# zihuixue/DynMM

Measured on AMD Instinct MI355X. Metric: images/sec fwd+bwd, 480x640 RGB-D, batch 32/GPU, higher is better.
Workload: dtype f32; 1 GPU; configs[2]: zero-grad + fwd + weighted 4-scale CE + FLOP loss + bwd + fused SGD-Nesterov update, --dynamic --global-gate soft DiffSoftmax gates tau=1; per_gpu_batch=32, global_batch=32, height=480, width=640, parallelism=dp1, launch=eager, streams=4, optimizer_in_step=fused SGD-Nesterov

## Files before the change

### dynmm_amd/csrc/common.h

```cpp
#pragma once
#include <hip/hip_runtime.h>
#include <stdint.h>
#include <stddef.h>

#include "dynmm_hip.h"

#if defined(__HIP_DEVICE_COMPILE__) && !defined(__gfx950__)
#error "libdynmm_hip is gfx950 (MI355X) code: build with --offload-arch=gfx950"
#endif

#define DYNMM_LAUNCH_CHECK()                                   \
    do {                                                       \
        hipError_t e__ = hipGetLastError();                    \
        if (e__ != hipSuccess) return -(1000 + (int)e__);      \
    } while (0)

#define DYNMM_HIP_TRY(expr)                                    \
    do {                                                       \
        hipError_t e__ = (expr);                               \
        if (e__ != hipSuccess) return -(1000 + (int)e__);      \
    } while (0)

namespace dynmm {

// ... 18 lines not shown
    return v;
}

template <typename T>
__device__ __forceinline__ T block_reduce_sum_256(T v, T* smem) {
    v = wave_reduce_sum(v);
    const int lane = threadIdx.x & 63, wave = threadIdx.x >> 6;
    __syncthreads();
    if (lane == 0) smem[wave] = v;
    __syncthreads();
    T r = T(0);
    if (threadIdx.x == 0) r = smem[0] + smem[1] + smem[2] + smem[3];
    return r;
}

__device__ __forceinline__ float sigmoid_f(float v) { return 1.f / (1.f + expf(-v)); }
__device__ __forceinline__ float swish_fwd(float v) { return v / (1.f + expf(-v)); }
__device__ __forceinline__ float hswish_fwd(float v) { return v * fminf(fmaxf(v + 3.f, 0.f), 6.f) / 6.f; }

__device__ __forceinline__ float act_fwd(float v, int act) {
    if (act == DYNMM_ACT_RELU) return v > 0.f ? v : 0.f;
    if (act == DYNMM_ACT_TANH) return tanhf(v);
    if (act == DYNMM_ACT_SWISH) return swish_fwd(v);
    if (act == DYNMM_ACT_HSWISH) return hswish_fwd(v);
    return v;
}

__device__ __forceinline__ float act_grad_pre(float z, int act) {
    if (act == DYNMM_ACT_RELU) return z > 0.f ? 1.f : 0.f;
    if (act == DYNMM_ACT_TANH) { const float t = tanhf(z); return 1.f - t * t; }
// ... 22 lines not shown
```

### dynmm_amd/csrc/norm.hip

```cpp
#include "common.h"
#include "vec.h"

namespace dynmm {

__device__ __forceinline__ size_t mask_word(int plane, int groups, int i) { return ((size_t)plane * groups + (i >> 8)) * 4; }

static inline int reduce_splits(int N, int C) {
    int s = 2048 / (C > 0 ? C : 1);
    if (s < 1) s = 1;
    if (s > N) s = N;
    return s;
}

template <int V>
__global__ void __launch_bounds__(256) bn_stats_kernel(const float* __restrict__ x,
                                                       double* __restrict__ sums,
                                                       int N, int C, int HW) {
    __shared__ float red[4];
    const int c = blockIdx.x, S = gridDim.y;
    float s1 = 0.f, s2 = 0.f;
    for (int n = blockIdx.y; n < N; n += S) {
        const float* p = x + ((size_t)n * C + c) * HW;
        float a1 = 0.f, a2 = 0.f;
        for (int i = threadIdx.x * V; i < HW; i += 256 * V) {
// ... 679 lines not shown
```

### dynmm_amd/csrc/pointwise.hip

```cpp
#include "common.h"
#include <initializer_list>
#include "vec.h"

namespace dynmm {

__device__ __forceinline__ float keep_if(float v, bool keep) { return __int_as_float(__float_as_int(v) & -(int)keep); }


static inline int plane_chunks(int HW, int chunk) { return (HW + chunk - 1) / chunk; }
constexpr int kChunk = 8192;

__global__ void __launch_bounds__(256) maxpool_fwd_kernel(const float* __restrict__ x,
                                                          float* __restrict__ y,
                                                          signed char* __restrict__ idx, int H,
                                                          int W, int Ho, int Wo) {
    const size_t plane = blockIdx.x;
    const float* xp = x + plane * H * W;
    const int HoWo = Ho * Wo;
    const int beg = blockIdx.y * kChunk, end = min(HoWo, beg + kChunk);
    for (int i = beg + threadIdx.x; i < end; i += 256) {
        const int oh = i / Wo, ow = i - oh * Wo;
        float best = -INFINITY;
        int bi = -1;
#pragma unroll
// ... 772 lines not shown
        for (int j = 0; j < V; ++j) acc[j] += v[j];
        if (n > 2) {
            vload<V>(S.p[2] + i, v);
#pragma unroll
            for (int j = 0; j < V; ++j) acc[j] += v[j];
        }
        if (n > 3) {
            vload<V>(S.p[3] + i, v);
#pragma unroll
            for (int j = 0; j < V; ++j) acc[j] += v[j];
        }
        vstore<V>(out + i, acc);
    }
}

}

using namespace dynmm;

#define ST ((hipStream_t)stream)

extern "C" int dynmm_add_n(const float* const* srcs, int n, float* out, size_t numel, void* stream) {
    (void)hipGetLastError();
    if (!srcs || !out || n < 2 || n > 4 || numel == 0) return DYNMM_EINVAL;
    AddSrcs S{};
    bool v4 = (numel % 4 == 0) && aligned16(out);
    for (int i = 0; i < n; ++i) {
        if (!srcs[i]) return DYNMM_EINVAL;
        S.p[i] = srcs[i];
        v4 = v4 && aligned16(srcs[i]);
    }
    size_t blocks = (numel / (v4 ? 4 : 1) + 255) / 256;
    if (blocks > 8192) blocks = 8192;
    if (blocks < 1) blocks = 1;
    if (v4)
        hipLaunchKernelGGL(add_n_kernel<4>, dim3((unsigned)blocks), dim3(256), 0, ST, S, n, out, numel);
    else
        hipLaunchKernelGGL(add_n_kernel<1>, dim3((unsigned)blocks), dim3(256), 0, ST, S, n, out, numel);
    DYNMM_LAUNCH_CHECK();
    return DYNMM_OK;
}

extern "C" int dynmm_batch_gather(const float* src, const int* idx, float* dst, int n_out, size_t row,
                                  void* stream) {
    (void)hipGetLastError();
    if (!src || !dst || n_out <= 0 || row == 0) return DYNMM_EINVAL;
    unsigned bx = (unsigned)((row / 4 + 255) / 256);
    if (bx > 64) bx = 64;
    if (bx < 1) bx = 1;
    if (row % 4 == 0 && aligned16(src) && aligned16(dst))
        hipLaunchKernelGGL(batch_gather_kernel<4>, dim3(bx, n_out), dim3(256), 0, ST, src, idx, dst, row);
    else
        hipLaunchKernelGGL(batch_gather_kernel<1>, dim3(bx, n_out), dim3(256), 0, ST, src, idx, dst, row);
// ... 213 lines not shown
        hipLaunchKernelGGL(axpby_bwd_reduce_kernel<1>, dim3(NC), dim3(256), 0, ST, g, xr, xd, da, db, HW);
    DYNMM_LAUNCH_CHECK();
    return DYNMM_OK;
}

extern "C" int dynmm_axpby_bwd_apply(const float* g, const float* a, const float* b, const float* ca,
                                     const float* cb, float cscale, float* dxr, float* dxd, int NC,
                                     int HW, void* stream) {
    (void)hipGetLastError();
    if (!g || !a || !b || !dxr || !dxd || NC <= 0 || HW <= 0) return DYNMM_EINVAL;
    dim3 grid(NC, plane_chunks(HW, kChunk));
    if (can_vec4(HW, {g, dxr, dxd}))
        hipLaunchKernelGGL(axpby_bwd_apply_kernel<4>, grid, dim3(256), 0, ST, g, a, b, ca, cb, cscale, dxr, dxd, HW);
    else
        hipLaunchKernelGGL(axpby_bwd_apply_kernel<1>, grid, dim3(256), 0, ST, g, a, b, ca, cb, cscale, dxr, dxd, HW);
    DYNMM_LAUNCH_CHECK();
    return DYNMM_OK;
}

namespace dynmm {

struct StemBnArgs {
    const float* go; const signed char* io;
    const float* gd; const signed char* id;
    const float* coef; const float* off; float cscale;
    const float* x; const float* mean; const float* invstd; const float* gamma; const float* beta;
    int N, C, H, W, Ho, Wo;
};

__device__ __forceinline__ void stem_gy_block(const StemBnArgs& a, size_t plane, int ar, int t, float fc, float fo,
// ... 199 lines not shown
```

### dynmm_amd/lib.py

```python
import ctypes as C
import os
import subprocess

_HERE = os.path.dirname(os.path.abspath(__file__))
LIB_PATH = os.path.join(_HERE, 'libdynmm_hip.so')
CSRC = os.path.join(_HERE, 'csrc')

ACT_NONE, ACT_RELU, ACT_TANH, ACT_SWISH, ACT_HSWISH = 0, 1, 2, 3, 4
SMOOTH_ACTS = (ACT_SWISH, ACT_HSWISH)
DYNMM_OK, DYNMM_EINVAL, DYNMM_EUNSUPPORTED, DYNMM_EWORKSPACE = 0, -1, -2, -3
ACT = {None: 0, 'none': 0, 'relu': 1, 'tanh': 2, 'swish': 3, 'silu': 3, 'hswish': 4}
LOSS_BCE_LOGITS, LOSS_L1 = 0, 1

c_f = C.c_void_p
c_i = C.c_int
c_fl = C.c_float
c_sz = C.c_size_t
c_ll = C.c_longlong


class ConvGeom(C.Structure):
    _fields_ = [(n, C.c_int) for n in ('N', 'Ci', 'H', 'W', 'Co', 'Ho', 'Wo',
                                       'KH', 'KW', 'SH', 'SW', 'PH', 'PW', 'c_split')]

# ... 80 lines not shown
    'dynmm_upsample2x_fwd': (c_i, [c_f] * 3 + [c_i] * 5 + [c_f]),
    'dynmm_upsample2x_bwd': (c_i, [c_f] * 2 + [c_i] * 5 + [c_f]),
    'dynmm_upsample2x_dw3x3_rep_fwd': (c_i, [c_f] * 5 + [c_i] * 4 + [c_f]),
    'dynmm_upsample2x_dw3x3_rep_bwd': (c_i, [c_f] * 7 + [c_i] * 4 + [c_f]),
    'dynmm_bilinear_into_fwd': (c_i, [c_f, c_f] + [c_i] * 8 + [c_f]),
    'dynmm_bilinear_into_bwd': (c_i, [c_f, c_f] + [c_i] * 8 + [c_f]),
    'dynmm_gap2_fwd': (c_i, [c_f] * 4 + [c_i, c_i, c_f]),
    'dynmm_se_coeff_fwd': (c_i, [c_f, c_f, _PP, c_f, c_i] + [c_f] * 6 + [c_i, c_i, c_i, c_f]),
    'dynmm_se_coeff_fwd_act': (c_i, [c_f, c_f, _PP, c_f, c_i] + [c_f] * 6 + [c_i, c_i, c_i, c_i, c_f]),
    'dynmm_se_coeff_bwd_act': (c_i, [c_f] * 4 + [_PP, c_f, c_i] + [c_f] * 4 + [_PP, c_f, c_f, c_f, c_i, c_f, c_i, c_i, c_i, c_i, c_f]),
    'dynmm_se_coeff_bwd_workspace_bytes': (c_sz, [c_i, c_i]),
    'dynmm_se_coeff_bwd': (c_i, [c_f] * 4 + [_PP, c_f, c_i] + [c_f] * 4 + [_PP, c_f, c_f, c_f, c_i, c_f, c_i, c_i, c_i, c_f]),
    'dynmm_axpby_fwd': (c_i, [c_f] * 5 + [c_i, c_i, c_f]),
    'dynmm_axpby_bwd_reduce': (c_i, [c_f] * 5 + [c_i, c_i, c_f]),
    'dynmm_axpby_bwd_apply': (c_i, [c_f] * 5 + [c_fl, c_f, c_f, c_i, c_i, c_f]),
    'dynmm_axpby_pool_supported': (c_i, [c_i, c_i]),
    'dynmm_axpby_pool_fwd': (c_i, [c_f] * 9 + [c_i] * 4 + [c_f]),
    'dynmm_axpby_pool_bwd_reduce': (c_i, [c_f] * 7 + [c_i] * 4 + [c_f]),
    'dynmm_stem_bn_bwd_reduce': (c_i, [c_f] * 6 + [c_fl] + [c_f] * 6 + [c_i] * 5 + [c_f]),
    'dynmm_stem_bn_bwd_apply': (c_i, [c_f] * 6 + [c_fl] + [c_f] * 9 + [c_i] * 4 + [c_f]),
    'dynmm_gap2_bnrelu_fwd': (c_i, [c_f] * 3 + [c_i] + [c_f] * 2 + [c_i] * 2 + [c_f]),
    'dynmm_bn_finalize': (c_i, [c_f] * 10 + [c_i] * 3 + [c_fl, c_fl, c_f]),
    'dynmm_axpby_pool_bwd_apply': (c_i, [c_f] * 8 + [C.c_float] + [c_f] * 2 + [c_i] * 3 + [c_f]),
    'dynmm_reweigh_fwd': (c_i, [c_f, c_f, _PP, c_f, c_i, c_f, c_i, c_f, C.c_ulonglong, C.c_ulonglong, c_fl, c_i]
                          + [c_f] * 6 + [c_i, c_i, c_f]),
    'dynmm_reweigh_fwd_act': (c_i, [c_f, c_f, _PP, c_f, c_i, c_f, c_i, c_f, C.c_ulonglong, C.c_ulonglong, c_fl, c_i]
                              + [c_f] * 6 + [c_i, c_i, c_i, c_f]),
    'dynmm_reweigh_bwd_act': (c_i, [c_f] * 5 + [_PP, c_f, c_i, c_f, c_f, c_f, _PP, c_f, c_f, c_f, c_f, c_f, c_fl, c_i, c_i, c_i,
                                    c_f]),
    'dynmm_reweigh_bwd_workspace_bytes': (c_sz, [c_i, c_i]),
    'dynmm_reweigh_bwd': (c_i, [c_f] * 5 + [_PP, c_f, c_i, c_f, c_f, c_f, _PP, c_f, c_f, c_f, c_f, c_f, c_fl, c_i, c_i, c_f]),
    'dynmm_gate_head_fwd': (c_i, [c_f] * 8 + [c_i, c_i, c_fl, c_i, c_i, c_f]),
    'dynmm_gate_decide': (c_i, [c_f] * 5 + [c_i, c_f]),
    'dynmm_gate_head_bwd': (c_i, [c_f] * 9 + [c_i, c_i, c_fl, c_f]),
    'dynmm_ce2d_fwd': (c_i, [c_f] * 4 + [c_i, c_i, c_i, c_i, c_f]),
    'dynmm_up2ce_fwd': (c_i, [c_f] * 7 + [c_i] * 5 + [c_f]),
    'dynmm_up2ce_bwd_workspace_bytes': (c_sz, [c_i] * 4),
    'dynmm_up2ce_bwd': (c_i, [c_f] * 11 + [c_i] * 4 + [c_f]),
    'dynmm_loss_head': (c_i, [c_f, c_i, c_f, c_fl, c_fl, c_f, c_f, c_f, c_f, c_f]),
    'dynmm_ce2d_valid': (c_i, [c_f] * 4 + [c_i, c_i, c_i, c_f]),
    'dynmm_ce2d_bwd': (c_i, [c_f] * 5 + [c_i, c_i, c_i, c_f]),
    'dynmm_eval_confusion': (c_i, [c_f, c_f, c_f] + [c_i] * 6 + [c_f]),
    'dynmm_batch_gather': (c_i, [c_f, c_f, c_f, c_i, c_sz, c_f]),
    'dynmm_batch_merge': (c_i, [c_f, c_f, c_f, c_f, c_i, c_sz, c_f]),
    'dynmm_add_n': (c_i, [_PP, c_i, c_f, c_sz, c_f]),
    'dynmm_reduce_slabs': (c_i, [c_f, c_f, c_i, c_i, c_f]),
    'dynmm_opt_tick': (c_i, [c_f, c_f]),
    'dynmm_sgd_nesterov': (c_i, [c_f, c_f, c_f, c_sz, c_sz, c_f, c_fl, c_fl, c_f, c_f, c_f, c_f]),
    'dynmm_adam': (c_i, [c_f, c_f, c_f, c_f, c_sz, c_sz, c_f, c_f, c_fl, c_fl, c_f, c_f, c_i, c_f, c_f]),
    'dynmm_layernorm_fwd': (c_i, [c_f] * 7 + [c_i, c_i, c_i, c_fl, c_f]),
    'dynmm_layernorm_bwd': (c_i, [c_f] * 9 + [c_i, c_i, c_i, c_f]),
    'dynmm_moe_blend_bwd': (c_i, [c_f, c_f, c_f, _PP, c_i, c_f, c_fl, _PP, c_f, c_i, c_f]),
    'dynmm_mha_fwd': (c_i, [c_f, c_f, c_f, c_i, c_i, c_i, c_i, c_f]),
    'dynmm_mha_bwd': (c_i, [c_f, c_f, c_f, c_f, c_i, c_i, c_i, c_i, c_f]),
    'dynmm_dropout_apply': (c_i, [c_f, c_f, c_sz, _DP, c_f]),
    'dynmm_layernorm_drop_fwd': (c_i, [c_f] * 7 + [c_i, c_i, c_i, c_fl, _DP, c_f]),
    'dynmm_layernorm_drop_bwd': (c_i, [c_f] * 10 + [c_i, c_i, c_i, _DP, c_f]),
    'dynmm_layernorm_bwd_workspace_bytes': (c_sz, [c_i, c_i, c_i]),
    'dynmm_layernorm_drop_bwd_ws': (c_i, [c_f] * 10 + [c_i, c_i, c_i, _DP, c_f, c_sz, c_f]),
    'dynmm_layernorm_parts_fwd': (c_i, [c_f, c_i] + [c_f] * 8 + [c_i, c_i, c_i, c_fl, _DP, c_f]),
# ... 101 lines not shown
```

### dynmm_amd/nn/blocks.py

```python
import torch
import torch.nn as nn

from .. import ops

ACTIVATIONS = {'relu': 'relu', 'swish': 'swish', 'silu': 'swish', 'hswish': 'hswish'}


def normalize_activation(activation):
    key = activation.lower() if isinstance(activation, str) else activation
    if key not in ACTIVATIONS:
        raise NotImplementedError('Only relu, swish and hswish as activation function are supported so far. '
                                  'Got {}'.format(activation))
    return ACTIVATIONS[key]


def conv_bn_act(x, conv, bn, act=None, residual=None, x2=None, mask_input=False, conv_link=None, res_link=None, bwd_link=None):
    if not bn.training and not torch.is_grad_enabled():
        return ops.conv2d_fused_eval(x, conv.weight, conv.bias, bn, act, residual,
                                     conv.stride, conv.padding, x2)
    y = ops.conv2d(x, conv.weight, conv.bias, conv.stride, conv.padding, None, x2, mask_input=mask_input, link=conv_link,
                   bn_stats=bn.training)
    return ops.batch_norm_act(y, bn, act, residual, link=res_link, bwd_link=bwd_link)


class ConvBNAct(nn.Sequential):

    def __init__(self, cin, cout, kernel_size, activation='relu'):
        super().__init__()
        self.activation = normalize_activation(activation)
        self.add_module('conv', nn.Conv2d(cin, cout, kernel_size, padding=kernel_size // 2, bias=False))
        self.add_module('bn', nn.BatchNorm2d(cout))

    def forward(self, x):
        return conv_bn_act(x, self.conv, self.bn, self.activation)


class NonBottleneck1D(nn.Module):
# ... 155 lines not shown
```

### dynmm_amd/nn/decoder.py

```python
import torch
import torch.nn as nn

from .. import ops
from .blocks import ConvBNAct, NonBottleneck1D, chain_ok


UPSAMPLING_MODES = ('nearest', 'bilinear', 'learned-3x3', 'learned-3x3-zeropad')


class Upsample(nn.Module):

    def __init__(self, mode='learned-3x3-zeropad', channels=None):
        super().__init__()
        if mode not in UPSAMPLING_MODES:
            raise NotImplementedError(f'Upsampling mode must be one of {UPSAMPLING_MODES}. Got {mode}')
        self.mode = mode
        if 'learned-3x3' in mode:
            self.pad = nn.Identity()
            self.conv = nn.Conv2d(channels, channels, 3, padding=1 if mode == 'learned-3x3-zeropad' else 0,
                                  groups=channels)
            k = torch.tensor([1., 2., 1.]) / 4
            with torch.no_grad():
                self.conv.weight.copy_((k[:, None] * k[None, :]).expand(channels, 1, 3, 3))
                self.conv.bias.zero_()
# ... 17 lines not shown
        self.encoder_decoder_fusion = encoder_decoder_fusion
        self.conv3x3 = ConvBNAct(channels_in, channels_dec, 3, activation)
        self.decoder_blocks = nn.Sequential(*[NonBottleneck1D(channels_dec, channels_dec, activation=activation)
                                              for _ in range(nr_decoder_blocks)])
        self.upsample = Upsample(upsampling_mode, channels_dec)
        self.side_output = nn.Conv2d(channels_dec, num_classes, 1)

    def forward(self, x, skip):
        y = self.conv3x3(x)
        blocks = list(self.decoder_blocks)
        for i, blk in enumerate(blocks):
            y = blk(y, chain=i > 0 and chain_ok(blocks[i - 1], blk))
        side = None
        if self.training:
            s = self.side_output
            y, ys = ops.fan_out(y, 2)
            side = ops.conv2d(ys, s.weight, s.bias, 1, 0)
        return self.upsample(y, skip if self.encoder_decoder_fusion == 'add' else None), side


class Decoder(nn.Module):
    def __init__(self, channels_in, channels_decoder, nr_decoder_blocks, num_classes,
                 upsampling_mode='learned-3x3-zeropad', encoder_decoder_fusion='add', activation='relu'):
        super().__init__()
        cd = channels_decoder
        kw = dict(upsampling_mode=upsampling_mode, encoder_decoder_fusion=encoder_decoder_fusion, activation=activation)
        self.decoder_module_1 = DecoderModule(channels_in, cd[0], nr_decoder_blocks[0], num_classes, **kw)
        self.decoder_module_2 = DecoderModule(cd[0], cd[1], nr_decoder_blocks[1], num_classes, **kw)
        self.decoder_module_3 = DecoderModule(cd[1], cd[2], nr_decoder_blocks[2], num_classes, **kw)
        self.conv_out = nn.Conv2d(cd[2], num_classes, 3, padding=1)
        self.upsample1 = Upsample(upsampling_mode, num_classes)
# ... 23 lines not shown
```

### dynmm_amd/nn/net.py

```python
import warnings

import numpy as np
import torch
import torch.nn as nn

from .. import ops
from .blocks import ConvBNAct, ResNetEncoder, conv_bn_act, normalize_activation
from .context import get_context_module
from .decoder import UPSAMPLING_MODES, Decoder
from .fusion import SqueezeAndExciteFusionAdd


def DiffSoftmax(logits, tau=1.0, hard=False, dim=-1):
    n = logits.shape[0]
    if logits.dim() < 2 or logits.shape[1] != 5 or logits.numel() != 5 * n or dim not in (1, 1 - logits.dim()):
        raise NotImplementedError('HIP DiffSoftmax handles [N,5] / [N,5,1,1] logits along dim 1')
    eye = torch.eye(5, device=logits.device, dtype=torch.float32)
    tab = torch.zeros(5, device=logits.device, dtype=torch.float32)
    w, _, _ = ops.gate_head(logits.reshape(n, 5), eye, tab, tau, hard)
    return w.reshape(logits.shape)


class GlobalGate(nn.Module):

# ... 282 lines not shown
                        d = getattr(ed, f'forward_layer{j}')(d_in)
                    fuse = ops.se_fuse_blend(r, d, self._se(j), wc, j - 1, inplace=True, se_act=self.activation)
                else:
                    r = getattr(er, f'forward_layer{j}')(r_in)
                    fuse, d = r, None
                if j < 4:
                    skips.append(decoder_skip(self, j, fuse))
        else:
            wcs = ops.fan_out(wcum, 4)
            for j in (1, 2, 3, 4):
                if self.dual_stream:
                    r, d = encoder_stage_pair(self, j, r if j == 1 else fuse, d)
                else:
                    r = getattr(er, f'forward_layer{j}')(r if j == 1 else fuse)
                    d = getattr(ed, f'forward_layer{j}')(d)
                d_f = d
                if j < 4:
                    d_f, d = ops.fan_out(d, 2)
                fuse = ops.se_fuse_blend(r, d_f, self._se(j), wcs[j - 1], j - 1, se_act=self.activation)
                if j < 4 and self.encoder_decoder_fusion == 'add':
                    fuse, f_skip = ops.fan_out(fuse, 2)
                    skips.append(decoder_skip(self, j, f_skip))
                elif j < 4:
                    skips.append(None)
        out = self.context_module(fuse)
        out = self.decoder([out, skips[2], skips[1], skips[0]], unpermute=unpermute)

        if test:
            return (out, weight) if return_weight else out
        return out, loss
```

### dynmm_amd/ops.py

```python
import contextlib
import ctypes as C

import torch
from torch.autograd import Function

from . import lib as L

ACT = L.ACT


def _lib():
    return L.load()


def _stream():
    if not torch.cuda.is_available():
        raise L.DynmmHipError('no HIP device is available: the DynMM hot path runs only on its HIP kernels '
                              '(there is no CPU / eager-PyTorch fallback)')
    h = torch.cuda.current_stream().cuda_stream
    _CENSUS.add(h)
    return h


def _p(t):
# ... 522 lines not shown
    __slots__ = ('dres',)

    def __init__(self):
        self.dres = None


class BNLink:
    __slots__ = ('x', 'mean', 'invstd', 'gamma', 'beta', 'sums', 'bits', 'premasked')

    def __init__(self):
        self.x = self.mean = self.invstd = self.gamma = self.beta = self.sums = self.bits = None
        self.premasked = False


BN_BWD_FUSE = True
BN_RELU_BITS = True


class PackedWeights:

    def __init__(self):
        self.reg = {}
        self.slots = {}
        self.arena = self.desc = self.wdesc = self.w43desc = self.w2desc = None
        self.blocks = self.wblocks = self.nwino = self.w43blocks = self.nw43 = self.w2blocks = self.nw2 = 0
        self.valid = False
        self.dirty = False

    def register(self, weight, g, need_fwd=True, need_dgrad=False, wino_fwd=False, wino_dgrad=False, wino43_dgrad=False,
                 wino2d_fwd=False, wino2d_dgrad=False):
# ... 354 lines not shown
    if not torch.is_grad_enabled() and isinstance(weight, torch.nn.Parameter) and w_owner is None:
        return conv2d_fused_eval(x, weight, bias, None, act, None, stride, padding, x2)
    holder = {} if (bn_stats and CONV_BN_STATS and x2 is None) else None
    y = _Conv2d.apply(x, x2, weight, bias, _pair(stride), _pair(padding), ACT[act], bool(mask_input),
                      bool(defer_mask), link, w_owner, holder, bn_link if BN_BWD_FUSE else None)
    if holder:
        y._bn_sums = holder['sums']
    if ACT_TRACE is not None and ACT[act] == L.ACT_RELU:
        ACT_TRACE.append(y.detach())
    return y


class _FanOut(Function):

    @staticmethod
    def forward(ctx, x, n):
        return tuple(x.view_as(x) for _ in range(n))

    @staticmethod
    def backward(ctx, *gs):
        gs = [_chk(g, 'grad') for g in gs if g is not None]
        if not gs:
            return None, None
        if len(gs) == 1:
            return gs[0], None
        out = torch.empty_like(gs[0])
        while len(gs) > 1:
            take, gs = gs[:4], gs[4:]
            dst = out if not gs else torch.empty_like(out)
            L.check(_lib().dynmm_add_n(_ptr_array(take), len(take), _p(dst), C.c_size_t(dst.numel()), _stream()), 'add_n')
            gs = [dst] + gs
        return out, None


_NO_FANOUT = False


def fan_out(x, n):
    if n <= 1 or _NO_FANOUT or not (torch.is_grad_enabled() and x.requires_grad):
        return (x,) * n
    return _FanOut.apply(x, n)


_MUTATION_GEN = [0]


def note_mutation():
    _MUTATION_GEN[0] += 1


CAPTURE_EVAL_CACHE = False


def conv2d_fused_eval(x, weight, conv_bias, bn, act=None, residual=None, stride=1, padding=0, x2=None):
    lib = _lib()
    st = _stream()
# ... 444 lines not shown
    if mode == 'nearest':
        return nearest_concat(x, *ys)
    if mode != 'bilinear':
        raise NotImplementedError(f'resize_concat: mode must be "nearest" or "bilinear", got {mode!r}')
    return _BilinearConcat.apply(x, *ys)


def _ptr_array(tensors):
    arr = (C.c_void_p * len(tensors))(*[t.data_ptr() for t in tensors])
    return arr


class _SEFuseBlend(Function):

    @staticmethod
    def forward(ctx, rgb, depth, wcum, col, use_se, inplace, se_act, *params):
        lib = _lib()
        st = _stream()
        rgb, depth = _chk(rgb, 'rgb'), _chk(depth, 'depth')
        N, Cc, H, W = rgb.shape
        n_act = depth.shape[0]
        if n_act > N or tuple(depth.shape[1:]) != tuple(rgb.shape[1:]) or n_act <= 0:
            raise L.DynmmHipError(f'rgb/depth fusion: shape mismatch {tuple(rgb.shape)} vs {tuple(depth.shape)}')
        HW = H * W
        dev = rgb.device
        f32 = dict(device=dev, dtype=torch.float32)
        wc_ptr, wc_stride = None, 0
        if wcum is not None:
            wcum = _chk(wcum, 'wcum')
            wc_stride = wcum.shape[1]
            wc_ptr = wcum.data_ptr() + 4 * col
        sr = sd = hr = hd = gr = gd = None
        parr = None
        if use_se:
            params = [_chk(p, 'se param') for p in params]
            parr = _ptr_array(params)
# ... 41 lines not shown
            parr, dparr = _ptr_array(params), _ptr_array(dparams)
            dsr, dsd = torch.empty((n_act, Cc), **f32), torch.empty((n_act, Cc), **f32)
        dwcum = None
        wc_ptr, wc_stride, dwc_ptr = None, 0, None
        if wcum is not None:
            wc_stride = wcum.shape[1]
            wc_ptr = wcum.data_ptr() + 4 * ctx.col
            if ctx.needs_input_grad[2]:
                dwcum = torch.zeros_like(wcum)
                dwc_ptr = dwcum.data_ptr() + 4 * ctx.col
        ws = torch.empty(lib.dynmm_se_coeff_bwd_workspace_bytes(n_act, Cc) // 4, **f32) if ctx.use_se else None
        L.check(lib.dynmm_se_coeff_bwd_act(_p(da), _p(db), _p(sr), _p(sd), parr, wc_ptr, wc_stride,
                                           _p(hr), _p(hd), _p(gr), _p(gd), dparr, _p(dsr), _p(dsd),
                                           dwc_ptr, wc_stride, _p(ws), n_act, Cc, int(ctx.use_se), ctx.se_act, st), 'se_coeff_bwd')
        drgb, ddepth = torch.empty_like(rgb), torch.empty_like(depth)
        L.check(lib.dynmm_axpby_bwd_apply(_p(g), _p(a), _p(b), _p(dsr), _p(dsd), 1.0 / HW,
                                          _p(drgb), _p(ddepth), n_act * Cc, HW, st), 'axpby_bwd_apply')
        _copy_rows(g, drgb, n_act, N - n_act)
        _grads_enqueued()
        return (drgb, ddepth, dwcum, None, None, None, None, *dparams_ret)


class _SEFusePool(Function):

    @staticmethod
    def forward(ctx, rgb, depth, use_se, se_act, *params):
        lib = _lib()
        st = _stream()
        rgb, depth = _chk(rgb, 'rgb'), _chk(depth, 'depth')
        _same_shape(rgb, depth, 'stem fusion')
        N, Cc, H, W = rgb.shape
        HW = H * W
        f32 = dict(device=rgb.device, dtype=torch.float32)
        sr = sd = hr = hd = gr = gd = None
        parr = None
# ... 214 lines not shown
def stem_bn_fuse_supported(h, w, bn_a, bn_b, act='relu'):
    return ACT[act] == L.ACT_RELU and _FUSED_STEM_BN and _FUSED_STEM_POOL and bool(_lib().dynmm_axpby_pool_supported(int(h), int(w))) and \
        bn_a.training and bn_b.training and torch.is_grad_enabled() and bn_a.momentum is not None and \
        bn_b.momentum is not None


def se_fuse_pool_supported(x):
    return _FUSED_STEM_POOL and x.dim() == 4 and bool(_lib().dynmm_axpby_pool_supported(int(x.shape[2]), int(x.shape[3])))


def se_fuse_pool(rgb, depth, se_params=None, se_act='relu'):
    use_se = se_params is not None
    return _SEFusePool.apply(rgb, depth, use_se, ACT[se_act], *(tuple(se_params) if use_se else ()))


def se_fuse_blend(rgb, depth, se_params=None, wcum=None, col=0, inplace=False, se_act='relu'):
    use_se = se_params is not None
    params = tuple(se_params) if use_se else ()
    return _SEFuseBlend.apply(rgb, depth, wcum, col, use_se, bool(inplace) and not torch.is_grad_enabled(), ACT[se_act], *params)


_PHILOX_OFFSET = [0]


def manual_seed(seed):
    global _PHILOX_SEED
    _PHILOX_SEED = int(seed) & 0xFFFFFFFFFFFFFFFF
    _PHILOX_OFFSET[0] = 0


_PHILOX_SEED = 0x5EEDD1CE


class _ReweighFuse(Function):
# ... 386 lines not shown
```

### include/dynmm_hip.h

```cpp
#ifndef DYNMM_HIP_H
#define DYNMM_HIP_H

#include <stddef.h>

#ifdef __cplusplus
extern "C" {
#endif

#define DYNMM_OK 0
#define DYNMM_EINVAL (-1)
#define DYNMM_EUNSUPPORTED (-2)
#define DYNMM_EWORKSPACE (-3)

#define DYNMM_ACT_NONE 0
#define DYNMM_ACT_RELU 1
#define DYNMM_ACT_TANH 2
#define DYNMM_ACT_SWISH 3
#define DYNMM_ACT_HSWISH 4

#define DYNMM_LOSS_BCE_LOGITS 0
#define DYNMM_LOSS_L1 1

int dynmm_abi_version(void);
const char* dynmm_build_info(void);
// ... 166 lines not shown
                           const float* wc, int wc_stride, float* a, float* b,
                           float* hr, float* hd, float* gr, float* gd,
                           int N, int C, int use_se, int act, void* stream);
int dynmm_se_coeff_bwd_act(const float* da, const float* db, const float* sr, const float* sd,
                           const float* const* params, const float* wc, int wc_stride,
                           const float* hr, const float* hd, const float* gr, const float* gd,
                           float* const* dparams, float* dsr, float* dsd, float* dwc, int dwc_stride,
                           float* workspace, int N, int C, int use_se, int act, void* stream);
int dynmm_axpby_fwd(const float* xr, const float* xd, const float* a, const float* b, float* out,
                    int NC, int HW, void* stream);
int dynmm_axpby_bwd_reduce(const float* g, const float* xr, const float* xd, float* da, float* db,
                           int NC, int HW, void* stream);
int dynmm_axpby_bwd_apply(const float* g, const float* a, const float* b,
                          const float* ca, const float* cb, float cscale, float* dxr, float* dxd,
                          int NC, int HW, void* stream);

int dynmm_axpby_pool_supported(int H, int W);
int dynmm_axpby_pool_fwd(const float* xr, const float* xd, const float* a, const float* b, float* y_out,
                         signed char* idx_out, float* y_depth, signed char* idx_depth, const float* bn_tr, int C,
                         int NC, int H, int W, void* stream);
int dynmm_axpby_pool_bwd_reduce(const float* g_out, const signed char* idx_out, const float* xr, const float* xd,
                                float* da, float* db, const float* bn_tr, int C, int NC, int H, int W, void* stream);
int dynmm_gap2_bnrelu_fwd(const float* xr, const float* xd, const float* bn_tr, int C, float* sr, float* sd, int NC,
                          int HW, void* stream);
int dynmm_stem_bn_bwd_reduce(const float* g_out, const signed char* idx_out, const float* g_depth,
                             const signed char* idx_depth, const float* coef, const float* off, float cscale,
                             const float* x, const float* mean, const float* invstd, const float* gamma,
                             const float* beta, double* sums, int N, int C, int H, int W, int sums_are_zero, void* stream);
int dynmm_stem_bn_bwd_apply(const float* g_out, const signed char* idx_out, const float* g_depth,
                            const signed char* idx_depth, const float* coef, const float* off, float cscale,
// ... 47 lines not shown
                    float* lse, double* loss_sum_wsum, int N, int C, int H, int W, int acc_is_zero, void* stream);
size_t dynmm_up2ce_bwd_workspace_bytes(int N, int C, int H, int W);
int dynmm_up2ce_bwd(const float* x, const float* w, const float* b, const unsigned char* target, const float* cw,
                    const float* lse, const float* gscale, float* dx, float* dw, float* db, float* workspace,
                    int N, int C, int H, int W, void* stream);

int dynmm_eval_confusion(const float* logits, const unsigned char* label, long long* cm,
                         int N, int C, int H, int W, int Ho, int Wo, void* stream);

int dynmm_batch_gather(const float* src, const int* idx, float* dst, int n_out, size_t row, void* stream);
int dynmm_gate_decide(const float* weight, int* branch, int* order, int* inv, int* counts, int N, void* stream);
int dynmm_batch_merge(const float* base, const float* sub, const int* map, float* out, int N, size_t row,
                      void* stream);

int dynmm_add_n(const float* const* srcs, int n, float* out, size_t numel, void* stream);
int dynmm_reduce_slabs(const float* slabs, float* out, int n, int nslabs, void* stream);
int dynmm_opt_tick(int* step, void* stream);
int dynmm_sgd_nesterov(float* p, const float* g, float* buf, size_t lo, size_t hi, const float* hyper,
                       float weight_decay, float grad_scale, const float* loss, int* nan_flag,
                       const int* step, void* stream);
int dynmm_adam(float* p, const float* g, float* m, float* v, size_t lo, size_t hi, const float* hyper,
               const int* step, float weight_decay, float grad_scale, const float* loss, int* nan_flag,
               int decoupled , const float* grad_scale_dev ,
               void* stream);

int dynmm_layernorm_fwd(const float* x, const float* res, const float* gamma, const float* beta, float* y,
                        float* mean, float* rstd, int B, int D, int T, float eps, void* stream);
int dynmm_layernorm_bwd(const float* g, const float* x, const float* res, const float* gamma, const float* mean,
                        const float* rstd, float* dx, float* dgamma, float* dbeta, int B, int D, int T, void* stream);
int dynmm_mha_fwd(const float* qkv, float* out, float* probs, int B, int D, int T, int heads, void* stream);
// ... 122 lines not shown
```

Baseline: 520.0 images/s.

## Fuse BN-backward reduction into fan-out grad sum and SE-blend backward apply

Measured after the change: 523.1 images/s (median of 6 runs). Within noise of the previous version (+0.6%).

```diff
diff --git a/dynmm_amd/csrc/common.h b/dynmm_amd/csrc/common.h
--- a/dynmm_amd/csrc/common.h
+++ b/dynmm_amd/csrc/common.h
@@ -56,6 +56,8 @@
     return r;
 }
 
+__device__ __forceinline__ size_t mask_word(int plane, int groups, int i) { return ((size_t)plane * groups + (i >> 8)) * 4; }
+
 __device__ __forceinline__ float sigmoid_f(float v) { return 1.f / (1.f + expf(-v)); }
 __device__ __forceinline__ float swish_fwd(float v) { return v / (1.f + expf(-v)); }
 __device__ __forceinline__ float hswish_fwd(float v) { return v * fminf(fmaxf(v + 3.f, 0.f), 6.f) / 6.f; }
diff --git a/dynmm_amd/csrc/norm.hip b/dynmm_amd/csrc/norm.hip
--- a/dynmm_amd/csrc/norm.hip
+++ b/dynmm_amd/csrc/norm.hip
@@ -3,7 +3,6 @@
 
 namespace dynmm {
 
-__device__ __forceinline__ size_t mask_word(int plane, int groups, int i) { return ((size_t)plane * groups + (i >> 8)) * 4; }
 
 static inline int reduce_splits(int N, int C) {
     int s = 2048 / (C > 0 ? C : 1);
diff --git a/dynmm_amd/csrc/pointwise.hip b/dynmm_amd/csrc/pointwise.hip
--- a/dynmm_amd/csrc/pointwise.hip
+++ b/dynmm_amd/csrc/pointwise.hip
@@ -810,6 +810,96 @@
     }
 }
 
+struct BnRedSide {
+    const float* x;
+    const float* mean;
+    const float* invstd;
+    const unsigned long long* bits;
+    double* sums;
+};
+
+__device__ __forceinline__ void bn_mask_reduce4(float (&g)[4], const float* __restrict__ xp,
+                                                const unsigned long long* __restrict__ w, int lane, float mu, float is,
+                                                float& s1, float& s2) {
+    float xv[4];
+    vload<4>(xp, xv);
+#pragma unroll
+    for (int j = 0; j < 4; ++j) {
+        const float ge = ((w[j] >> lane) & 1ull) ? g[j] : 0.f;
+        g[j] = ge;
+        s1 += ge;
+        s2 += ge * (xv[j] - mu) * is;
+    }
+}
+
+__device__ __forceinline__ void bn_red_commit(float s1, float s2, float* red, double* __restrict__ sums, int c, int C) {
+    const float t1 = block_reduce_sum_256<float>(s1, red);
+    const float t2 = block_reduce_sum_256<float>(s2, red);
+    if (threadIdx.x == 0) {
+        atomicAdd(&sums[c], (double)t1);
+        atomicAdd(&sums[C + c], (double)t2);
+    }
+}
+
+__global__ void __launch_bounds__(256) add_n_bnred_kernel(AddSrcs S, int n, BnRedSide r, float* __restrict__ out, int C, int HW) {
+    __shared__ float red[4];
+    const int plane = blockIdx.x, c = plane % C;
+    const float mu = r.mean[c], is = r.invstd[c];
+    const int groups = (HW + 255) >> 8, lane = threadIdx.x & 63;
+    const size_t base = (size_t)plane * HW;
+    const int beg = blockIdx.y * kChunk, end = min(HW, beg + kChunk);
+    float s1 = 0.f, s2 = 0.f;
+    for (int i = beg + threadIdx.x * 4; i < end; i += 256 * 4) {
+        float acc[4], v[4];
+        vload<4>(S.p[0] + base + i, acc);
+        vload<4>(S.p[1] + base + i, v);
+#pragma unroll
+        for (int j = 0; j < 4; ++j) acc[j] += v[j];
+        if (n > 2) {
+            vload<4>(S.p[2] + base + i, v);
+#pragma unroll
+            for (int j = 0; j < 4; ++j) acc[j] += v[j];
+        }
+        if (n > 3) {
+            vload<4>(S.p[3] + base + i, v);
+#pragma unroll
+            for (int j = 0; j < 4; ++j) acc[j] += v[j];
+        }
+        bn_mask_reduce4(acc, r.x + base + i, r.bits + mask_word(plane, groups, i), lane, mu, is, s1, s2);
+        vstore<4>(out + base + i, acc);
+    }
+    bn_red_commit(s1, s2, red, r.sums, c, C);
+}
+
+__global__ void __launch_bounds__(256) axpby_bwd_apply_bnred_kernel(
+    const float* __restrict__ g, const float* __restrict__ a, const float* __restrict__ b,
+    const float* __restrict__ ca, const float* __restrict__ cb, float cscale,
+    float* __restrict__ dxr, float* __restrict__ dxd, BnRedSide rr, BnRedSide rd, int C, int HW) {
+    __shared__ float red[4];
+    const int plane = blockIdx.x, c = plane % C;
+    const size_t base = (size_t)plane * HW;
+    const float fa = a[plane], fb = b[plane];
+    const float oa = ca ? ca[plane] * cscale : 0.f, ob = cb ? cb[plane] * cscale : 0.f;
+    const float mur = rr.x ? rr.mean[c] : 0.f, isr = rr.x ? rr.invstd[c] : 0.f;
+    const float mud = rd.x ? rd.mean[c] : 0.f, isd = rd.x ? rd.invstd[c] : 0.f;
+    const int groups = (HW + 255) >> 8, lane = threadIdx.x & 63;
+    const int beg = blockIdx.y * kChunk, end = min(HW, beg + kChunk);
+    float r1 = 0.f, r2 = 0.f, d1 = 0.f, d2 = 0.f;
+    for (int i = beg + threadIdx.x * 4; i < end; i += 256 * 4) {
+        float gv[4], r[4], d[4];
+        vload<4>(g + base + i, gv);
+#pragma unroll
+        for (int j = 0; j < 4; ++j) { r[j] = fa * gv[j] + oa; d[j] = fb * gv[j] + ob; }
+        const size_t w = mask_word(plane, groups, i);
+        if (rr.x) bn_mask_reduce4(r, rr.x + base + i, rr.bits + w, lane, mur, isr, r1, r2);
+        if (rd.x) bn_mask_reduce4(d, rd.x + base + i, rd.bits + w, lane, mud, isd, d1, d2);
+        vstore<4>(dxr + base + i, r);
+        vstore<4>(dxd + base + i, d);
+    }
+    if (rr.x) bn_red_commit(r1, r2, red, rr.sums, c, C);
+    if (rd.x) bn_red_commit(d1, d2, red, rd.sums, c, C);
+}
+
 }
 
 using namespace dynmm;
@@ -833,6 +923,31 @@
         hipLaunchKernelGGL(add_n_kernel<4>, dim3((unsigned)blocks), dim3(256), 0, ST, S, n, out, numel);
     else
         hipLaunchKernelGGL(add_n_kernel<1>, dim3((unsigned)blocks), dim3(256), 0, ST, S, n, out, numel);
+    DYNMM_LAUNCH_CHECK();
+    return DYNMM_OK;
+}
+
+static bool bnred_side_ok(const BnRedSide& r) {
+    return r.x && r.mean && r.invstd && r.bits && r.sums && aligned16(r.x) && (reinterpret_cast<uintptr_t>(r.bits) & 7u) == 0;
+}
+
+extern "C" int dynmm_add_n_bnred(const float* const* srcs, int n, const float* x, const float* mean, const float* invstd,
+                                 const unsigned long long* relu_bits, double* sums, int sums_are_zero, float* out, int N,
+                                 int C, int HW, void* stream) {
+    (void)hipGetLastError();
+    if (!srcs || !out || n < 2 || n > 4 || !x || !mean || !invstd || !relu_bits || !sums || N <= 0 || C <= 0 || HW <= 0)
+        return DYNMM_EINVAL;
+    AddSrcs S{};
+    bool ok = HW % 4 == 0 && aligned16(out);
+    for (int i = 0; i < n; ++i) {
+        if (!srcs[i]) return DYNMM_EINVAL;
+        S.p[i] = srcs[i];
+        ok = ok && aligned16(srcs[i]);
+    }
+    const BnRedSide r{x, mean, invstd, relu_bits, sums};
+    if (!ok || !bnred_side_ok(r)) return DYNMM_EUNSUPPORTED;
+    if (!sums_are_zero) DYNMM_HIP_TRY(hipMemsetAsync(sums, 0, sizeof(double) * 2 * C, ST));
+    hipLaunchKernelGGL(add_n_bnred_kernel, dim3(N * C, plane_chunks(HW, kChunk)), dim3(256), 0, ST, S, n, r, out, C, HW);
     DYNMM_LAUNCH_CHECK();
     return DYNMM_OK;
 }
@@ -1076,6 +1191,28 @@
         hipLaunchKernelGGL(axpby_bwd_apply_kernel<4>, grid, dim3(256), 0, ST, g, a, b, ca, cb, cscale, dxr, dxd, HW);
     else
         hipLaunchKernelGGL(axpby_bwd_apply_kernel<1>, grid, dim3(256), 0, ST, g, a, b, ca, cb, cscale, dxr, dxd, HW);
+    DYNMM_LAUNCH_CHECK();
+    return DYNMM_OK;
+}
+
+extern "C" int dynmm_axpby_bwd_apply_bnred(const float* g, const float* a, const float* b, const float* ca, const float* cb,
+                                           float cscale, float* dxr, float* dxd, const float* x_r, const float* mean_r,
+                                           const float* invstd_r, const unsigned long long* bits_r, double* sums_r,
+                                           const float* x_d, const float* mean_d, const float* invstd_d,
+                                           const unsigned long long* bits_d, double* sums_d, int sums_are_zero, int N, int C,
+                                           int HW, void* stream) {
+    (void)hipGetLastError();
+    if (!g || !a || !b || !dxr || !dxd || N <= 0 || C <= 0 || HW <= 0 || (!x_r && !x_d) ||
+        (x_r && (!mean_r || !invstd_r || !bits_r || !sums_r)) || (x_d && (!mean_d || !invstd_d || !bits_d || !sums_d)))
+        return DYNMM_EINVAL;
+    const BnRedSide rr{x_r, mean_r, invstd_r, bits_r, sums_r}, rd{x_d, mean_d, invstd_d, bits_d, sums_d};
+    if (!can_vec4(HW, {g, dxr, dxd}) || (x_r && !bnred_side_ok(rr)) || (x_d && !bnred_side_ok(rd))) return DYNMM_EUNSUPPORTED;
+    if (!sums_are_zero) {
+        if (x_r) DYNMM_HIP_TRY(hipMemsetAsync(sums_r, 0, sizeof(double) * 2 * C, ST));
+        if (x_d) DYNMM_HIP_TRY(hipMemsetAsync(sums_d, 0, sizeof(double) * 2 * C, ST));
+    }
+    hipLaunchKernelGGL(axpby_bwd_apply_bnred_kernel, dim3(N * C, plane_chunks(HW, kChunk)), dim3(256), 0, ST, g, a, b, ca, cb,
+                       cscale, dxr, dxd, rr, rd, C, HW);
     DYNMM_LAUNCH_CHECK();
     return DYNMM_OK;
 }
diff --git a/dynmm_amd/lib.py b/dynmm_amd/lib.py
--- a/dynmm_amd/lib.py
+++ b/dynmm_amd/lib.py
@@ -118,6 +118,7 @@
     'dynmm_axpby_fwd': (c_i, [c_f] * 5 + [c_i, c_i, c_f]),
     'dynmm_axpby_bwd_reduce': (c_i, [c_f] * 5 + [c_i, c_i, c_f]),
     'dynmm_axpby_bwd_apply': (c_i, [c_f] * 5 + [c_fl, c_f, c_f, c_i, c_i, c_f]),
+    'dynmm_axpby_bwd_apply_bnred': (c_i, [c_f] * 5 + [c_fl, c_f, c_f] + [c_f] * 10 + [c_i] * 4 + [c_f]),
     'dynmm_axpby_pool_supported': (c_i, [c_i, c_i]),
     'dynmm_axpby_pool_fwd': (c_i, [c_f] * 9 + [c_i] * 4 + [c_f]),
     'dynmm_axpby_pool_bwd_reduce': (c_i, [c_f] * 7 + [c_i] * 4 + [c_f]),
@@ -148,6 +149,7 @@
     'dynmm_batch_gather': (c_i, [c_f, c_f, c_f, c_i, c_sz, c_f]),
     'dynmm_batch_merge': (c_i, [c_f, c_f, c_f, c_f, c_i, c_sz, c_f]),
     'dynmm_add_n': (c_i, [_PP, c_i, c_f, c_sz, c_f]),
+    'dynmm_add_n_bnred': (c_i, [_PP, c_i] + [c_f] * 5 + [c_i, c_f] + [c_i] * 3 + [c_f]),
     'dynmm_reduce_slabs': (c_i, [c_f, c_f, c_i, c_i, c_f]),
     'dynmm_opt_tick': (c_i, [c_f, c_f]),
     'dynmm_sgd_nesterov': (c_i, [c_f, c_f, c_f, c_sz, c_sz, c_f, c_fl, c_fl, c_f, c_f, c_f, c_f]),
diff --git a/dynmm_amd/nn/blocks.py b/dynmm_amd/nn/blocks.py
--- a/dynmm_amd/nn/blocks.py
+++ b/dynmm_amd/nn/blocks.py
@@ -21,6 +21,13 @@
     y = ops.conv2d(x, conv.weight, conv.bias, conv.stride, conv.padding, None, x2, mask_input=mask_input, link=conv_link,
                    bn_stats=bn.training)
     return ops.batch_norm_act(y, bn, act, residual, link=res_link, bwd_link=bwd_link)
+
+
+def tail_link(out, blk):
+    import torch.nn.modules.module as M
+    if blk._forward_hooks or M._global_forward_hooks or M._global_forward_pre_hooks:
+        return None
+    return getattr(out, '_bn_out_link', None)
 
 
 class ConvBNAct(nn.Sequential):
diff --git a/dynmm_amd/nn/decoder.py b/dynmm_amd/nn/decoder.py
--- a/dynmm_amd/nn/decoder.py
+++ b/dynmm_amd/nn/decoder.py
@@ -2,7 +2,7 @@
 import torch.nn as nn
 
 from .. import ops
-from .blocks import ConvBNAct, NonBottleneck1D, chain_ok
+from .blocks import ConvBNAct, NonBottleneck1D, chain_ok, tail_link
 
 
 UPSAMPLING_MODES = ('nearest', 'bilinear', 'learned-3x3', 'learned-3x3-zeropad')
@@ -55,7 +55,7 @@
         side = None
         if self.training:
             s = self.side_output
-            y, ys = ops.fan_out(y, 2)
+            y, ys = ops.fan_out(y, 2, bn_link=tail_link(y, blocks[-1]) if blocks else None)
             side = ops.conv2d(ys, s.weight, s.bias, 1, 0)
         return self.upsample(y, skip if self.encoder_decoder_fusion == 'add' else None), side
 
diff --git a/dynmm_amd/nn/net.py b/dynmm_amd/nn/net.py
--- a/dynmm_amd/nn/net.py
+++ b/dynmm_amd/nn/net.py
@@ -5,7 +5,7 @@
 import torch.nn as nn
 
 from .. import ops
-from .blocks import ConvBNAct, ResNetEncoder, conv_bn_act, normalize_activation
+from .blocks import ConvBNAct, ResNetEncoder, conv_bn_act, normalize_activation, tail_link
 from .context import get_context_module
 from .decoder import UPSAMPLING_MODES, Decoder
 from .fusion import SqueezeAndExciteFusionAdd
@@ -320,10 +320,14 @@
                 else:
                     r = getattr(er, f'forward_layer{j}')(r if j == 1 else fuse)
                     d = getattr(ed, f'forward_layer{j}')(d)
+                r_link = tail_link(r, getattr(er, f'layer{j}')[-1])
+                d_link = tail_link(d, getattr(ed, f'layer{j}')[-1])
                 d_f = d
                 if j < 4:
-                    d_f, d = ops.fan_out(d, 2)
-                fuse = ops.se_fuse_blend(r, d_f, self._se(j), wcs[j - 1], j - 1, se_act=self.activation)
+                    d_f, d = ops.fan_out(d, 2, bn_link=d_link)
+                    d_link = None
+                fuse = ops.se_fuse_blend(r, d_f, self._se(j), wcs[j - 1], j - 1, se_act=self.activation,
+                                         bn_links=(r_link, d_link))
                 if j < 4 and self.encoder_decoder_fusion == 'add':
                     fuse, f_skip = ops.fan_out(fuse, 2)
                     skips.append(decoder_skip(self, j, f_skip))
diff --git a/dynmm_amd/ops.py b/dynmm_amd/ops.py
--- a/dynmm_amd/ops.py
+++ b/dynmm_amd/ops.py
@@ -560,6 +560,17 @@
 
 
 BN_BWD_FUSE = True
+BN_TAIL_FUSE = {'fanout', 'blend'}
+
+
+def _tail_fuse(which):
+    return BN_BWD_FUSE and which in BN_TAIL_FUSE
+
+
+def _bnred_link(bl, like):
+    if bl is None or bl.x is None or bl.bits is None or bl.sums is not None or tuple(bl.x.shape) != tuple(like.shape):
+        return None
+    return bl
 BN_RELU_BITS = True
 
 
@@ -944,32 +955,43 @@
 class _FanOut(Function):
 
     @staticmethod
-    def forward(ctx, x, n):
+    def forward(ctx, x, n, bn_link=None):
+        ctx.bn_link = bn_link
         return tuple(x.view_as(x) for _ in range(n))
 
     @staticmethod
     def backward(ctx, *gs):
         gs = [_chk(g, 'grad') for g in gs if g is not None]
         if not gs:
-            return None, None
+            return None, None, None
         if len(gs) == 1:
-            return gs[0], None
+            return gs[0], None, None
         out = torch.empty_like(gs[0])
+        bl = _bnred_link(ctx.bn_link, out) if out.dim() == 4 else None
         while len(gs) > 1:
             take, gs = gs[:4], gs[4:]
             dst = out if not gs else torch.empty_like(out)
+            if bl is not None and not gs:
+                N, Cc, H, W = out.shape
+                sums, zeroed = _zero_sums(2 * Cc, out.device)
+                rc = _lib().dynmm_add_n_bnred(_ptr_array(take), len(take), _p(bl.x), _p(bl.mean), _p(bl.invstd), _p(bl.bits),
+                                              _p(sums), zeroed, _p(dst), N, Cc, H * W, _stream())
+                if rc != L.DYNMM_EUNSUPPORTED:
+                    L.check(rc, 'add_n_bnred')
+                    bl.sums, bl.premasked = sums, True
+                    break
             L.check(_lib().dynmm_add_n(_ptr_array(take), len(take), _p(dst), C.c_size_t(dst.numel()), _stream()), 'add_n')
             gs = [dst] + gs
-        return out, None
+        return out, None, None
 
 
 _NO_FANOUT = False
 
 
-def fan_out(x, n):
+def fan_out(x, n, bn_link=None):
     if n <= 1 or _NO_FANOUT or not (torch.is_grad_enabled() and x.requires_grad):
         return (x,) * n
-    return _FanOut.apply(x, n)
+    return _FanOut.apply(x, n, bn_link if _tail_fuse('fanout') else None)
 
 
 _MUTATION_GEN = [0]
@@ -1444,12 +1466,13 @@
 class _SEFuseBlend(Function):
 
     @staticmethod
-    def forward(ctx, rgb, depth, wcum, col, use_se, inplace, se_act, *params):
+    def forward(ctx, rgb, depth, wcum, col, use_se, inplace, se_act, bn_links, *params):
         lib = _lib()
         st = _stream()
         rgb, depth = _chk(rgb, 'rgb'), _chk(depth, 'depth')
         N, Cc, H, W = rgb.shape
         n_act = depth.shape[0]
+        ctx.bn_links = bn_links if (bn_links is not None and n_act == N) else (None, None)
         if n_act > N or tuple(depth.shape[1:]) != tuple(rgb.shape[1:]) or n_act <= 0:
             raise L.DynmmHipError(f'rgb/depth fusion: shape mismatch {tuple(rgb.shape)} vs {tuple(depth.shape)}')
         HW = H * W
@@ -1521,11 +1544,29 @@
                                            _p(hr), _p(hd), _p(gr), _p(gd), dparr, _p(dsr), _p(dsd),
                                            dwc_ptr, wc_stride, _p(ws), n_act, Cc, int(ctx.use_se), ctx.se_act, st), 'se_coeff_bwd')
         drgb, ddepth = torch.empty_like(rgb), torch.empty_like(depth)
-        L.check(lib.dynmm_axpby_bwd_apply(_p(g), _p(a), _p(b), _p(dsr), _p(dsd), 1.0 / HW,
-                                          _p(drgb), _p(ddepth), n_act * Cc, HW, st), 'axpby_bwd_apply')
+        lr, ld = (_bnred_link(bl, rgb) for bl in ctx.bn_links)
+        fused = False
+        if lr is not None or ld is not None:
+            side = []
+            for bl in (lr, ld):
+                sums = _zero_sums(2 * Cc, g.device) if bl is not None else (None, 1)
+                side.append((bl, sums[0], sums[1]))
+            desc = [p_ for bl, sums, _ in side for p_ in
+                    ((_p(bl.x), _p(bl.mean), _p(bl.invstd), _p(bl.bits), _p(sums)) if bl is not None else (None,) * 5)]
+            rc = lib.dynmm_axpby_bwd_apply_bnred(_p(g), _p(a), _p(b), _p(dsr), _p(dsd), 1.0 / HW, _p(drgb), _p(ddepth), *desc,
+                                                 int(all(z for _, _, z in side)), N, Cc, HW, st)
+            if rc != L.DYNMM_EUNSUPPORTED:
+                L.check(rc, 'axpby_bwd_apply_bnred')
+                fused = True
+                for bl, sums, _ in side:
+                    if bl is not None:
+                        bl.sums, bl.premasked = sums, True
+        if not fused:
+            L.check(lib.dynmm_axpby_bwd_apply(_p(g), _p(a), _p(b), _p(dsr), _p(dsd), 1.0 / HW,
+                                              _p(drgb), _p(ddepth), n_act * Cc, HW, st), 'axpby_bwd_apply')
         _copy_rows(g, drgb, n_act, N - n_act)
         _grads_enqueued()
-        return (drgb, ddepth, dwcum, None, None, None, None, *dparams_ret)
+        return (drgb, ddepth, dwcum, None, None, None, None, None, *dparams_ret)
 
 
 class _SEFusePool(Function):
@@ -1770,10 +1811,13 @@
     return _SEFusePool.apply(rgb, depth, use_se, ACT[se_act], *(tuple(se_params) if use_se else ()))
 
 
-def se_fuse_blend(rgb, depth, se_params=None, wcum=None, col=0, inplace=False, se_act='relu'):
+def se_fuse_blend(rgb, depth, se_params=None, wcum=None, col=0, inplace=False, se_act='relu', bn_links=None):
     use_se = se_params is not None
     params = tuple(se_params) if use_se else ()
-    return _SEFuseBlend.apply(rgb, depth, wcum, col, use_se, bool(inplace) and not torch.is_grad_enabled(), ACT[se_act], *params)
+    if bn_links is not None and not (_tail_fuse('blend') and torch.is_grad_enabled() and any(bl is not None for bl in bn_links)):
+        bn_links = None
+    return _SEFuseBlend.apply(rgb, depth, wcum, col, use_se, bool(inplace) and not torch.is_grad_enabled(), ACT[se_act],
+                              tuple(bn_links) if bn_links is not None else None, *params)
 
 
 _PHILOX_OFFSET = [0]
diff --git a/include/dynmm_hip.h b/include/dynmm_hip.h
--- a/include/dynmm_hip.h
+++ b/include/dynmm_hip.h
@@ -204,6 +204,13 @@
 int dynmm_axpby_bwd_apply(const float* g, const float* a, const float* b,
                           const float* ca, const float* cb, float cscale, float* dxr, float* dxd,
                           int NC, int HW, void* stream);
+int dynmm_axpby_bwd_apply_bnred(const float* g, const float* a, const float* b, const float* ca, const float* cb,
+                                float cscale, float* dxr, float* dxd,
+                                const float* x_r, const float* mean_r, const float* invstd_r,
+                                const unsigned long long* bits_r, double* sums_r,
+                                const float* x_d, const float* mean_d, const float* invstd_d,
+                                const unsigned long long* bits_d, double* sums_d,
+                                int sums_are_zero, int N, int C, int HW, void* stream);
 
 int dynmm_axpby_pool_supported(int H, int W);
 int dynmm_axpby_pool_fwd(const float* xr, const float* xd, const float* a, const float* b, float* y_out,
@@ -281,6 +288,9 @@
                       void* stream);
 
 int dynmm_add_n(const float* const* srcs, int n, float* out, size_t numel, void* stream);
+int dynmm_add_n_bnred(const float* const* srcs, int n, const float* x, const float* mean, const float* invstd,
+                      const unsigned long long* relu_bits, double* sums, int sums_are_zero, float* out,
+                      int N, int C, int HW, void* stream);
 int dynmm_reduce_slabs(const float* slabs, float* out, int n, int nslabs, void* stream);
 int dynmm_opt_tick(int* step, void* stream);
 int dynmm_sgd_nesterov(float* p, const float* g, float* buf, size_t lo, size_t hi, const float* hyper,
```
